# tangxyw/RecAlgorithm

Measured on AMD Instinct MI355X. Metric: CTR examples/sec (train step fwd+bwd+TF1-Adam), batch 4096/GPU, 26 fields x emb16, higher is better.
Workload: dtype f32; 1 GPU; DCN 3-layer CrossNet + MLP 512,256,128; 26 fields x emb16; batch 4096/GPU; data_batches=32, global_batch=4096, fields=26, emb_dim=16, embedding_rows=2790871, launch=hipGraph replay, parallelism=single

## Files before the change

recalgorithm_amd/csrc/cross_bwd.h:

```cpp
#pragma once
#include "common.h"

namespace recalgo_cross {

template <int N>
__device__ __forceinline__ void wave_sum_n(float (&v)[N]) {
#pragma unroll
    for (int o = 32; o > 0; o >>= 1) {
        float t[N];
#pragma unroll
        for (int i = 0; i < N; ++i) t[i] = __shfl_xor(v[i], o, 64);
#pragma unroll
        for (int i = 0; i < N; ++i) v[i] += t[i];
    }
}

template <int NV, int L, int WAVES>
__device__ __forceinline__ void cross_stack_bwd_block(
    const float* __restrict__ x0, unsigned x_stride, const float4* __restrict__ w,
    const float4* __restrict__ b, const float* __restrict__ g, unsigned g_stride,
    const float* __restrict__ g_x0_extra, unsigned B, unsigned d4, float* __restrict__ dx0,
    float* __restrict__ partials, unsigned block, unsigned nblocks, float* smem) {
    constexpr int kBwdWaves = WAVES, kBwdThreads = WAVES * 64;
    const unsigned lane = threadIdx.x & 63;
    const unsigned wib = threadIdx.x >> 6;
    const unsigned wave = block * kBwdWaves + wib;
    const unsigned nwaves = nblocks * kBwdWaves;
    const unsigned d = d4 * 4;

    float4 wv[L][NV];
    float beta_part[L];
    {
        float4 Bv[NV];
#pragma unroll
        for (int v = 0; v < NV; ++v) Bv[v] = f4_zero();
#pragma unroll
        for (int l = 0; l < L; ++l) {
            float acc = 0.f;
#pragma unroll
            for (int v = 0; v < NV; ++v) {
                unsigned idx = lane + v * 64;
                wv[l][v] = idx < d4 ? w[l * d4 + idx] : f4_zero();
                acc += f4_dot(Bv[v], wv[l][v]);
                if (idx < d4) Bv[v] = f4_add(Bv[v], b[l * d4 + idx]);
            }
            beta_part[l] = acc;
        }
    }
    float4 A[L][NV], G[NV];
    float T[L];
#pragma unroll
    for (int v = 0; v < NV; ++v) G[v] = f4_zero();
#pragma unroll
    for (int l = 0; l < L; ++l) {
        T[l] = 0.f;
#pragma unroll
        for (int v = 0; v < NV; ++v) A[l][v] = f4_zero();
    }

    for (unsigned ex = wave; ex < B; ex += nwaves) {
        const float4* xr = reinterpret_cast<const float4*>(x0 + (size_t)ex * x_stride);
        const float4* gr = reinterpret_cast<const float4*>(g + (size_t)ex * g_stride);
        float4 xv[NV], gv[NV];
#pragma unroll
        for (int v = 0; v < NV; ++v) {
            unsigned idx = lane + v * 64;
            xv[v] = idx < d4 ? xr[idx] : f4_zero();
            gv[v] = idx < d4 ? gr[idx] : f4_zero();
        }
        float r[2 * L + 1];
        {
            float q = 0.f;
#pragma unroll
            for (int v = 0; v < NV; ++v) q += f4_dot(gv[v], xv[v]);
            r[2 * L] = q;
        }
#pragma unroll
        for (int l = 0; l < L; ++l) {
            float acc = 0.f;
#pragma unroll
            for (int v = 0; v < NV; ++v) acc += f4_dot(xv[v], wv[l][v]);
            r[l] = acc;
            r[L + l] = beta_part[l];
        }
        wave_sum_n<2 * L + 1>(r);
        float c[L + 1];
        c[0] = 1.f;
#pragma unroll
        for (int l = 0; l < L; ++l) c[l + 1] = c[l] + fmaf(c[l], r[l], r[L + l]);
        float dc = r[2 * L];
        float dp[L];
#pragma unroll
        for (int l = L - 1; l >= 0; --l) {
            T[l] += dc;
            dp[l] = dc * c[l];
            dc = dc * (1.f + r[l]);
        }
        float4* orow = reinterpret_cast<float4*>(dx0 + (size_t)ex * x_stride);
#pragma unroll
        for (int v = 0; v < NV; ++v) {
            unsigned idx = lane + v * 64;
            float4 o = f4_scale(gv[v], c[L]);
#pragma unroll
            for (int l = 0; l < L; ++l) {
                o = f4_fma(wv[l][v], dp[l], o);
                A[l][v] = f4_fma(xv[v], dp[l], A[l][v]);
            }
            G[v] = f4_add(G[v], gv[v]);
            if (idx < d4) {
                if (g_x0_extra)
                    o = f4_add(o, reinterpret_cast<const float4*>(g_x0_extra + (size_t)ex * x_stride)[idx]);
                orow[idx] = o;
            }
        }
    }

    const unsigned row_len = 2 * L * d;
    float* prow = partials + (size_t)block * row_len;
    float* sT = smem + (size_t)kBwdWaves * d;
    const float* wf = reinterpret_cast<const float*>(w);
    const float* bf = reinterpret_cast<const float*>(b);
    if (lane == 0) {
#pragma unroll
        for (int l = 0; l < L; ++l) sT[wib * L + l] = T[l];
    }
    __syncthreads();
    if (threadIdx.x < L) {
        float acc = 0.f;
        for (int wv_ = 0; wv_ < kBwdWaves; ++wv_) acc += sT[wv_ * L + threadIdx.x];
        sT[kBwdWaves * L + threadIdx.x] = acc;
    }
    __syncthreads();
    float Tw[L];
#pragma unroll
    for (int l = 0; l < L; ++l) Tw[l] = sT[kBwdWaves * L + l];
#pragma unroll
    for (int vec = 0; vec <= L; ++vec) {
        __syncthreads();
#pragma unroll
        for (int v = 0; v < NV; ++v) {
            unsigned idx = lane + v * 64;
            if (idx < d4) {
                float4 val = G[v];
#pragma unroll
                for (int l = 0; l < L; ++l)
                    if (vec == l) val = A[l][v];
                *reinterpret_cast<float4*>(smem + (size_t)wib * d + idx * 4) = val;
            }
        }
        __syncthreads();
        for (unsigned j = threadIdx.x; j < d; j += kBwdThreads) {
            float acc = 0.f;
#pragma unroll
            for (int wv_ = 0; wv_ < kBwdWaves; ++wv_) acc += smem[(size_t)wv_ * d + j];
            if (vec < L) {
                float Bl = 0.f;
#pragma unroll
                for (int jj = 0; jj < L; ++jj)
                    if (jj < vec) Bl += bf[(size_t)jj * d + j];
                prow[(size_t)vec * d + j] = fmaf(Bl, Tw[vec], acc);
            } else {
                float tail = 0.f;
#pragma unroll
                for (int jj = L - 1; jj >= 0; --jj) {
                    prow[(size_t)(L + jj) * d + j] = acc + tail;
                    tail = fmaf(Tw[jj], wf[(size_t)jj * d + j], tail);
                }
            }
        }
    }
}


}
```

Baseline: 20.44 million examples/s.

## Software-prefetch cross backward rows via register ring and preload weight columns

Adds a register ring buffer that issues the loads for the x0 and gradient rows one or two examples ahead, so global memory latency overlaps the per-example cross-layer compute. The prefetch depth depends on NV and L. For small NV it also loads the bias and weight column values into registers before the main loop, so the final partial-reduction phase no longer re-reads them from global memory. The cost is higher register pressure, which may lower occupancy.

```diff
diff --git a/recalgorithm_amd/csrc/cross_bwd.h b/recalgorithm_amd/csrc/cross_bwd.h
--- a/recalgorithm_amd/csrc/cross_bwd.h
+++ b/recalgorithm_amd/csrc/cross_bwd.h
@@ -28,6 +28,21 @@
     const unsigned nwaves = nblocks * kBwdWaves;
     const unsigned d = d4 * 4;
 
+    constexpr int kPrefetch = NV > 2 ? 0 : (NV * L > 6 ? 1 : 2), kRing = kPrefetch + 1;
+    float4 xring[kRing][NV], gring[kRing][NV];
+    auto request = [&](int slot, unsigned long long e) {
+        if (e >= B) return;
+        const float4* xr = reinterpret_cast<const float4*>(x0 + (size_t)e * x_stride);
+        const float4* gr = reinterpret_cast<const float4*>(g + (size_t)e * g_stride);
+#pragma unroll
+        for (int v = 0; v < NV; ++v) {
+            unsigned idx = lane + v * 64;
+            xring[slot][v] = idx < d4 ? xr[idx] : f4_zero();
+            gring[slot][v] = idx < d4 ? gr[idx] : f4_zero();
+        }
+    };
+#pragma unroll
+    for (int p = 0; p < kPrefetch; ++p) request(p, (unsigned long long)wave + (unsigned long long)p * nwaves);
     float4 wv[L][NV];
     float beta_part[L];
     {
@@ -47,6 +62,22 @@
             beta_part[l] = acc;
         }
     }
+    constexpr bool kEarlyCols = NV <= 2;
+    constexpr int kCols = (NV * 256 + kBwdThreads - 1) / kBwdThreads;
+    const float* wf = reinterpret_cast<const float*>(w);
+    const float* bf = reinterpret_cast<const float*>(b);
+    float bcol[kEarlyCols ? L : 1][kCols], wcol[kEarlyCols ? L : 1][kCols];
+    if constexpr (kEarlyCols) {
+#pragma unroll
+        for (int k = 0; k < kCols; ++k) {
+            const unsigned j = threadIdx.x + k * kBwdThreads;
+#pragma unroll
+            for (int l = 0; l < L; ++l) {
+                bcol[l][k] = j < d ? bf[(size_t)l * d + j] : 0.f;
+                wcol[l][k] = j < d ? wf[(size_t)l * d + j] : 0.f;
+            }
+        }
+    }
     float4 A[L][NV], G[NV];
     float T[L];
 #pragma unroll
@@ -58,16 +89,7 @@
         for (int v = 0; v < NV; ++v) A[l][v] = f4_zero();
     }
 
-    for (unsigned ex = wave; ex < B; ex += nwaves) {
-        const float4* xr = reinterpret_cast<const float4*>(x0 + (size_t)ex * x_stride);
-        const float4* gr = reinterpret_cast<const float4*>(g + (size_t)ex * g_stride);
-        float4 xv[NV], gv[NV];
-#pragma unroll
-        for (int v = 0; v < NV; ++v) {
-            unsigned idx = lane + v * 64;
-            xv[v] = idx < d4 ? xr[idx] : f4_zero();
-            gv[v] = idx < d4 ? gr[idx] : f4_zero();
-        }
+    auto example = [&](unsigned ex, const float4 (&xv)[NV], const float4 (&gv)[NV]) {
         float r[2 * L + 1];
         {
             float q = 0.f;
@@ -113,13 +135,20 @@
                 orow[idx] = o;
             }
         }
+    };
+    for (unsigned long long ex = wave; ex < B;) {
+#pragma unroll
+        for (int s = 0; s < kRing; ++s) {
+            if (ex >= B) break;
+            request((s + kPrefetch) % kRing, ex + (unsigned long long)kPrefetch * nwaves);
+            example((unsigned)ex, xring[s], gring[s]);
+            ex += nwaves;
+        }
     }
 
     const unsigned row_len = 2 * L * d;
     float* prow = partials + (size_t)block * row_len;
     float* sT = smem + (size_t)kBwdWaves * d;
-    const float* wf = reinterpret_cast<const float*>(w);
-    const float* bf = reinterpret_cast<const float*>(b);
     if (lane == 0) {
 #pragma unroll
         for (int l = 0; l < L; ++l) sT[wib * L + l] = T[l];
@@ -149,7 +178,7 @@
             }
         }
         __syncthreads();
-        for (unsigned j = threadIdx.x; j < d; j += kBwdThreads) {
+        auto column = [&](int k, unsigned j) {
             float acc = 0.f;
 #pragma unroll
             for (int wv_ = 0; wv_ < kBwdWaves; ++wv_) acc += smem[(size_t)wv_ * d + j];
@@ -157,16 +186,25 @@
                 float Bl = 0.f;
 #pragma unroll
                 for (int jj = 0; jj < L; ++jj)
-                    if (jj < vec) Bl += bf[(size_t)jj * d + j];
+                    if (jj < vec) Bl += kEarlyCols ? bcol[kEarlyCols ? jj : 0][k] : bf[(size_t)jj * d + j];
                 prow[(size_t)vec * d + j] = fmaf(Bl, Tw[vec], acc);
             } else {
                 float tail = 0.f;
 #pragma unroll
                 for (int jj = L - 1; jj >= 0; --jj) {
                     prow[(size_t)(L + jj) * d + j] = acc + tail;
-                    tail = fmaf(Tw[jj], wf[(size_t)jj * d + j], tail);
+                    tail = fmaf(Tw[jj], kEarlyCols ? wcol[kEarlyCols ? jj : 0][k] : wf[(size_t)jj * d + j], tail);
                 }
             }
+        };
+        if constexpr (kEarlyCols) {
+#pragma unroll
+            for (int k = 0; k < kCols; ++k) {
+                const unsigned j = threadIdx.x + k * kBwdThreads;
+                if (j < d) column(k, j);
+            }
+        } else {
+            for (unsigned j = threadIdx.x; j < d; j += kBwdThreads) column(0, j);
         }
     }
 }
```

Result: no change. 20.56 million examples/s (median of 6 runs) (+0.6%).
